# hanmekim/SceneLib2

Measured on AMD Instinct MI355X. Metric: batched MonoSLAM frames/sec (320x240, 100 feat), higher is better.
Workload: dtype f64

## Files before the change

scenelib2_amd/csrc/sl2_ekf_update.hip:

```cpp
#include "sl2_common.hpp"
#include "sl2_chol_diag.hpp"

namespace sl2 {

typedef double v4d __attribute__((ext_vector_type(4)));

__device__ __forceinline__ v4d mfma_f64(double a, double b, v4d c) {
  return __builtin_amdgcn_mfma_f64_16x16x4f64(a, b, c, 0, 0, 0);
}

#ifdef SL2_TESTING
#define SL2_EKF_TEST_SECTION 1
#include "sl2_ekf_update_testing.inc"
#undef SL2_EKF_TEST_SECTION
#endif

constexpr int kASBatch = 4;

template <int NQ, int BATCH>
__global__ void __launch_bounds__(1024) k_build_AS(const double* __restrict__ P, const double* __restrict__ f_Hx,
                                                  const double* __restrict__ f_Hy, const double* __restrict__ f_nu,
                                                  const double* __restrict__ f_R, const int* __restrict__ succ_idx,
                                                  const int* __restrict__ m_count, double* __restrict__ At,
                                                  double* __restrict__ St, const int* __restrict__ f_hcol,
                                                  const int* __restrict__ pos_err_any, int N, int ld, int mld) {
  extern __shared__ double sAt[];
  const int b = blockIdx.x;
  const int cnt = m_count[b];
  if (cnt == 0) return;
  const int m = 2 * cnt, mp = (m + 31) / 32 * 32;
  const int t = threadIdx.x;
  double* Ab = At + (size_t)b * mld * ld;
  double* Sb = St + (size_t)b * mld * mld;
  const double* Pb = P + (size_t)b * ld * ld;
// ... 101 lines not shown
  return r;
}
__device__ __forceinline__ double fast_rsqrt(double p) {
  double y = __builtin_amdgcn_rsq(p);
  y = y * __builtin_fma(-0.5 * p * y, y, 1.5);
  y = y * __builtin_fma(-0.5 * p * y, y, 1.5);
  return y;
}


#ifdef SL2_TESTING
#define SL2_EKF_TEST_SECTION 4
#include "sl2_ekf_update_testing.inc"
#undef SL2_EKF_TEST_SECTION
#endif

#ifdef SL2_TESTING
#define SL2_EKF_TEST_SECTION 5
#include "sl2_ekf_update_testing.inc"
#undef SL2_EKF_TEST_SECTION
#endif

#ifdef SL2_TESTING
#define SL2_EKF_TEST_SECTION 6
#include "sl2_ekf_update_testing.inc"
#undef SL2_EKF_TEST_SECTION
#endif


struct Tile32 {
  v4d f[2][2];
};

__device__ __forceinline__ Tile32 tile_load(const double* __restrict__ Sb, int mld, int k0, int i0, int lo, int hi) {
  Tile32 t;
#pragma unroll
  for (int kt = 0; kt < 2; ++kt)
#pragma unroll
    for (int it = 0; it < 2; ++it)
#pragma unroll
      for (int r = 0; r < 4; ++r) t.f[kt][it][r] = Sb[(size_t)(k0 + 16 * kt + hi + 4 * r) * mld + i0 + 16 * it + lo];
  return t;
}
__device__ __forceinline__ void tile_store(double* __restrict__ Sb, int mld, int k0, int i0, int lo, int hi, const Tile32& t) {
#pragma unroll
  for (int kt = 0; kt < 2; ++kt)
#pragma unroll
    for (int it = 0; it < 2; ++it)
#pragma unroll
      for (int r = 0; r < 4; ++r) Sb[(size_t)(k0 + 16 * kt + hi + 4 * r) * mld + i0 + 16 * it + lo] = t.f[kt][it][r];
}
constexpr int kTileAll = 15, kTileRowsLo = 5, kTileDiag = 11, kTileDiagLo = 1;
__device__ __forceinline__ Tile32 tile_panel(const double* sLinv, const double* __restrict__ Sb, int mld, int o, int i0, int lo,
                                             int hi, int need) {
  double b0[8], b1[8];
#pragma unroll
  for (int s8 = 0; s8 < 8; ++s8) {
    b0[s8] = Sb[(size_t)(o + 4 * s8 + hi) * mld + i0 + lo];
    b1[s8] = (need & 10) ? Sb[(size_t)(o + 4 * s8 + hi) * mld + i0 + 16 + lo] : 0.0;
  }
  Tile32 t;
#pragma unroll
  for (int kt = 0; kt < 2; ++kt)
#pragma unroll
    for (int it = 0; it < 2; ++it) t.f[kt][it] = (v4d){0, 0, 0, 0};
#pragma unroll
  for (int s8 = 0; s8 < 8; ++s8) {
    const int p = 4 * s8 + hi;
    const double a0 = sLinv[p * kLinvPitch + lo], a1 = sLinv[p * kLinvPitch + 16 + lo];
    t.f[0][0] = mfma_f64(a0, b0[s8], t.f[0][0]);
    if (need & 2) t.f[0][1] = mfma_f64(a0, b1[s8], t.f[0][1]);
    t.f[1][0] = mfma_f64(a1, b0[s8], t.f[1][0]);
    if (need & 8) t.f[1][1] = mfma_f64(a1, b1[s8], t.f[1][1]);
  }
  return t;
}
__device__ __forceinline__ Tile32 tile_panel_regs(const double* sLinv, const Tile32& in, int lo, int hi, int need) {
  Tile32 t;
#pragma unroll
  for (int kt = 0; kt < 2; ++kt)
#pragma unroll
    for (int it = 0; it < 2; ++it) t.f[kt][it] = (v4d){0, 0, 0, 0};
#pragma unroll
  for (int s8 = 0; s8 < 8; ++s8) {
    const int p = 4 * s8 + hi;
    const double a0 = sLinv[p * kLinvPitch + lo], a1 = sLinv[p * kLinvPitch + 16 + lo];
    const double b0 = in.f[s8 >> 2][0][s8 & 3], b1 = in.f[s8 >> 2][1][s8 & 3];
    t.f[0][0] = mfma_f64(a0, b0, t.f[0][0]);
    if (need & 2) t.f[0][1] = mfma_f64(a0, b1, t.f[0][1]);
    t.f[1][0] = mfma_f64(a1, b0, t.f[1][0]);
    if (need & 8) t.f[1][1] = mfma_f64(a1, b1, t.f[1][1]);
  }
  return t;
}
__device__ __forceinline__ void tile_trail(double* __restrict__ Sb, int mld, int o, int K, int I, int lo, int hi) {
  Tile32 acc = tile_load(Sb, mld, K * 32, I * 32, lo, hi);
#pragma unroll
  for (int h = 0; h < 2; ++h) {
    double a0[4], a1[4], b0[4], b1[4];
#pragma unroll
    for (int s4 = 0; s4 < 4; ++s4) {
      const size_t row = (size_t)(o + 16 * h + 4 * s4 + hi) * mld;
      a0[s4] = Sb[row + K * 32 + lo];
      a1[s4] = Sb[row + K * 32 + 16 + lo];
      b0[s4] = Sb[row + I * 32 + lo];
      b1[s4] = Sb[row + I * 32 + 16 + lo];
    }
#pragma unroll
    for (int s4 = 0; s4 < 4; ++s4) {
      acc.f[0][0] = mfma_f64(-a0[s4], b0[s4], acc.f[0][0]);
      acc.f[0][1] = mfma_f64(-a0[s4], b1[s4], acc.f[0][1]);
      acc.f[1][0] = mfma_f64(-a1[s4], b0[s4], acc.f[1][0]);
      acc.f[1][1] = mfma_f64(-a1[s4], b1[s4], acc.f[1][1]);
    }
  }
  tile_store(Sb, mld, K * 32, I * 32, lo, hi, acc);
}


#undef TR

__device__ __forceinline__ Tile32 tile_left_update(double* __restrict__ Sb, int mld, int J, int I, int kend, int lo, int hi, int need) {
  Tile32 acc = tile_load(Sb, mld, J * 32, I * 32, lo, hi);
  for (int K = 0; K < kend; ++K) {
#pragma unroll
    for (int h = 0; h < 2; ++h) {
      double a0[4], a1[4], b0[4], b1[4];
#pragma unroll
      for (int s4 = 0; s4 < 4; ++s4) {
        const size_t row = (size_t)(K * 32 + 16 * h + 4 * s4 + hi) * mld;
        a0[s4] = Sb[row + J * 32 + lo];
        a1[s4] = (need & 12) ? Sb[row + J * 32 + 16 + lo] : 0.0;
        b0[s4] = Sb[row + I * 32 + lo];
        b1[s4] = (need & 10) ? Sb[row + I * 32 + 16 + lo] : 0.0;
      }
#pragma unroll
      for (int s4 = 0; s4 < 4; ++s4) {
        acc.f[0][0] = mfma_f64(-a0[s4], b0[s4], acc.f[0][0]);
        if (need & 2) acc.f[0][1] = mfma_f64(-a0[s4], b1[s4], acc.f[0][1]);
        if (need & 4) acc.f[1][0] = mfma_f64(-a1[s4], b0[s4], acc.f[1][0]);
        if (need & 8) acc.f[1][1] = mfma_f64(-a1[s4], b1[s4], acc.f[1][1]);
      }
    }
  }
  return acc;
}
__device__ __forceinline__ void tile_diag_sub_regs(Tile32& acc, const Tile32& l, int need) {
#pragma unroll
  for (int s8 = 0; s8 < 8; ++s8) {
    const double v0 = l.f[s8 >> 2][0][s8 & 3], v1 = l.f[s8 >> 2][1][s8 & 3];
    acc.f[0][0] = mfma_f64(-v0, v0, acc.f[0][0]);
    if (need & 2) acc.f[0][1] = mfma_f64(-v0, v1, acc.f[0][1]);
    if (need & 4) acc.f[1][0] = mfma_f64(-v1, v0, acc.f[1][0]);
    if (need & 8) acc.f[1][1] = mfma_f64(-v1, v1, acc.f[1][1]);
  }
}

__global__ void __launch_bounds__(256, 4) k_chol_left(double* __restrict__ St, double* __restrict__ LinvT,
                                                      const int* __restrict__ m_count, int mld, int nblk_max, int J0, int nb_cap,
                                                      long long* trace) {
  const int b = blockIdx.x;
  const int cnt = m_count[b];
  if (cnt == 0) return;
  int nblk = (2 * cnt + 31) / 32 - J0;
  if (nblk <= 0) return;
  if (nblk > nb_cap) nblk = nb_cap;
  const int lane = threadIdx.x & 63, wave = threadIdx.x >> 6;
  const bool isD = wave == 0;
  const int mw = wave - 1;
  const bool half_last = 2 * cnt - 32 * (J0 + nblk - 1) <= 16;
  auto off_need = [&](int I) { return (half_last && I == nblk - 1) ? kTileRowsLo : kTileAll; };
  auto diag_need = [&](int I) { return (half_last && I == nblk - 1) ? kTileDiagLo : kTileDiag; };
  __shared__ double sTile[32][33];
  __shared__ double sLinv[32 * kLinvPitch];
  __shared__ double sNext[1024];
  __shared__ __attribute__((aligned(16))) double sCol[2][64];
  __shared__ double sIdent[32][33];
  double* Sb = St + (size_t)b * mld * mld + (size_t)J0 * 32 * mld + J0 * 32;
  LinvT += (size_t)J0 * 1024;
#ifdef SL2_CHOL_TRACE
#define TRL(slot) do { if (trace && lane == 0 && J < 8) trace[(((size_t)b * 4 + wave) * 8 + J) * 4 + (slot)] = (long long)__builtin_readcyclecounter(); } while (0)
#else
#define TRL(slot) do { } while (0)
#endif
#ifdef SL2_CHOL_TRACE
  if (trace && lane == 0) trace[(size_t)gridDim.x * 4 * 8 * 4 + b * 4 + wave] = __builtin_amdgcn_s_getreg(63492);
#endif
  auto diag_to_lds = [&](const Tile32& t, int lo, int hi) {
#pragma unroll
    for (int jt = 0; jt < 2; ++jt)
#pragma unroll
      for (int it = 0; it < 2; ++it)
#pragma unroll
        for (int r4 = 0; r4 < 4; ++r4) sTile[16 * it + lo][16 * jt + hi + 4 * r4] = t.f[jt][it][r4];
  };
  if (mw == 0) diag_to_lds(tile_load(Sb, mld, 0, 0, lane & 15, lane >> 4), lane & 15, lane >> 4);
  for (int i = threadIdx.x; i < 32 * 33; i += 256) (&sIdent[0][0])[i] = (i / 33 == i % 33) ? 1.0 : 0.0;
  __syncthreads();
  for (int J = 0; J < nblk; ++J) {
    const int o = J * 32;
    int lane_j = lane;
    asm volatile("" : "+v"(lane_j));
    const int lo = lane_j & 15, hi = lane_j >> 4;
    const bool more = J + 1 < nblk;
    TRL(0);
    TRL(1);
    auto solve_stored = [&](int turn) {
      for (int sidx = turn; ; sidx += 3) {
        const int t = sidx == 0 ? 3 : sidx + 4;
        if (J + t >= nblk) break;
        const Tile32 u = tile_panel(sLinv, Sb, mld, o, (J + t) * 32, lo, hi, off_need(J + t));
        tile_store(Sb, mld, o, (J + t) * 32, lo, hi, u);
      }
    };
    if (isD) {
      __builtin_amdgcn_s_setprio(3);
      const int r = lane_j & 31;
      const bool low = lane_j < 32;
      double a[32];
      const double* src = low ? &sTile[r][0] : &sIdent[r][0];
#pragma unroll
      for (int c = 0; c < 32; ++c) a[c] = src[c];
      double* rows = low ? &sTile[r][0] : &sLinv[r * kLinvPitch];
      DScal t;
      t.s = 0.0;
      d_column<0>(a, t, (unsigned)(size_t)(__attribute__((address_space(3))) double*)&sCol[0][0], &sCol[0][lane_j], rows);
      rows[31] = a[31];
      __builtin_amdgcn_s_setprio(0);
      TRL(2);
      __syncthreads();
      solve_stored(0);
    } else {
      Tile32 kept;
#pragma unroll
      for (int q = 0; q < 4; ++q) kept.f[q >> 1][q & 1] = (v4d){0, 0, 0, 0};
      int keptI = nblk;
      if (more) {
        if (mw == 1) {
          const Tile32 dn = tile_left_update(Sb, mld, J + 1, J + 1, J, lo, hi, diag_need(J + 1));
#pragma unroll
          for (int k = 0; k < 16; ++k) sNext[k * 64 + lane_j] = dn.f[k >> 3][(k >> 2) & 1][k & 3];
        }
        const int t_keep = mw == 0 ? 0 : (mw == 1 ? 4 : 2);
        for (int t = t_keep + 3; J + t < nblk; t += 3) {
          const Tile32 u = tile_left_update(Sb, mld, J, J + t, J, lo, hi, off_need(J + t));
          tile_store(Sb, mld, o, (J + t) * 32, lo, hi, u);
        }
        keptI = mw == 0 ? J + 1 : J + t_keep;
        if (keptI < nblk) kept = tile_left_update(Sb, mld, J, keptI, J, lo, hi, off_need(keptI));
      }
      TRL(2);
      __syncthreads();
      if (keptI < nblk) {
        const Tile32 l = tile_panel_regs(sLinv, kept, lo, hi, off_need(keptI));
        tile_store(Sb, mld, o, keptI * 32, lo, hi, l);
        if (mw == 0) {
          Tile32 dn;
#pragma unroll
          for (int q = 0; q < 16; ++q) dn.f[q >> 3][(q >> 2) & 1][q & 3] = sNext[q * 64 + lane_j];
          tile_diag_sub_regs(dn, l, diag_need(J + 1));
          diag_to_lds(dn, lo, hi);
        }
      }
      if (mw == 2) {
        double* Lb = LinvT + ((size_t)b * nblk_max + J) * 1024;
#pragma unroll
        for (int q = 0; q < 16; ++q) Lb[q * 64 + lane_j] = sLinv[(q * 2 + (lane_j >> 5)) * kLinvPitch + (lane_j & 31)];
      }
      if (mw >= 1) solve_stored(mw);
    }
    TRL(3);
    if (more) __syncthreads();
  }
}
#undef TRL

#ifdef SL2_TESTING
#define SL2_EKF_TEST_SECTION 8
#include "sl2_ekf_update_testing.inc"
#undef SL2_EKF_TEST_SECTION
#endif

constexpr int kFwdPitch = 48;

template <int NB>
__global__ void __launch_bounds__(256, (NB <= 8 ? 3 : 2)) k_fwdsub_lds(const double* At, double* Vt,
                                                    const double* St, const double* __restrict__ LinvT,
                                                    const int* __restrict__ m_count, int ld, int mld, int nblk_max, int B,
                                                    int J0, int col0, int ntile, int nb_cap) {
  int b, ct;
  if (!xcd_map(ntile, B, &b, &ct)) return;
  const int cnt = m_count[b];
  if (cnt == 0) return;
  int m = 2 * cnt - 32 * J0;
  if (m <= 0) return;
  if (m > 32 * nb_cap) m = 32 * nb_cap;
  const int nblk = (m + 31) / 32;
  const int tid = threadIdx.x, lane = tid & 63, wave = tid >> 6;
  const int lo = lane & 15, hi = lane >> 4;
  const int i0 = col0 + ct * 64 + wave * 16;
  const double* Ab = At + (size_t)b * mld * ld + (size_t)J0 * 32 * ld;
  double* Vb = Vt + (size_t)b * mld * ld + (size_t)J0 * 32 * ld;
  const double* Sb = St + (size_t)b * mld * mld + (size_t)J0 * 32 * mld + J0 * 32;
  const double* Lb = LinvT + ((size_t)b * nblk_max + J0) * 1024;
  __shared__ double sL[2][32 * kFwdPitch];
// ... 296 lines not shown
  const int cnt = m_count[b];
  if (cnt == 0) return;
  const int mp = (2 * cnt + 31) / 32 * 32;
  int ti = 0;
  while (t > ti) { t -= ti + 1; ++ti; }
  const int tj = t;
  const int j0 = c0 + tj * 64, i0 = c0 + ti * 64;
  if (j0 >= mp || i0 >= mp) return;
  const int tid = threadIdx.x, lane = tid & 63, wave = tid >> 6;
  const int lo = lane & 15, hi = lane >> 4;
  const int wj = (wave >> 1) * 32, wi = (wave & 1) * 32;
  double* Sb = St + (size_t)b * mld * mld;
  __shared__ double sAB[2][2][kSyrkKC * 64];
  v4d acc[2][2];
  for (int a = 0; a < 2; ++a) for (int c = 0; c < 2; ++c) acc[a][c] = (v4d){0, 0, 0, 0};
  const int kvalid = (mp - k0 < kp) ? mp - k0 : kp;
  const bool idle = (ti == tj) && (wj > wi);
  kpanel_product(Sb + (size_t)k0 * mld + j0, (size_t)mld, Sb + (size_t)k0 * mld + i0, (size_t)mld, kvalid / kSyrkKC, idle, wj, wi, sAB,
                 acc);
  if (idle) return;
#pragma unroll
  for (int a = 0; a < 2; ++a)
#pragma unroll
    for (int c = 0; c < 2; ++c)
#pragma unroll
      for (int r = 0; r < 4; ++r) {
        double* q = Sb + (size_t)(j0 + wj + 16 * a + hi + 4 * r) * mld + i0 + wi + 16 * c + lo;
        *q -= acc[a][c][r];
      }
}

constexpr int kCholPanelBlocks = 4;

static int launch_chol_panels(sl2_engine* e, int B) {
  const int pb = e->root->chol_panel == 8 ? 8 : kCholPanelBlocks;
  for (int p0 = 0; p0 < e->nblk_max; p0 += pb) {
    const int nb = e->nblk_max - p0 < pb ? e->nblk_max - p0 : pb;
    {
      LaunchScope ls(e, "k_chol_left", true);
      hipLaunchKernelGGL(k_chol_left, dim3(B), dim3(256), 0, e->stream, e->St, e->LinvT, e->m_gate, e->mld, e->nblk_max, p0, nb,
                         (long long*)nullptr);
      SL2_HIP(hipGetLastError());
    }
    const int c0 = (p0 + nb) * 32;
    if (c0 >= e->mld) break;
    const int ntile = (e->mld - c0) / 64;
    {
      LaunchScope ls(e, "k_fwdsub_lds@chol", true);
      if (pb == 8)
        hipLaunchKernelGGL((k_fwdsub_lds<8>), dim3(xcd_grid(ntile, B)), dim3(256), 0, e->stream, e->St, e->St, e->St,
                           e->LinvT, e->m_gate, e->mld, e->mld, e->nblk_max, B, p0, c0, ntile, nb);
      else
        hipLaunchKernelGGL((k_fwdsub_lds<kCholPanelBlocks>), dim3(xcd_grid(ntile, B)), dim3(256), 0, e->stream, e->St, e->St, e->St,
                           e->LinvT, e->m_gate, e->mld, e->mld, e->nblk_max, B, p0, c0, ntile, nb);
      SL2_HIP(hipGetLastError());
    }
    {
      LaunchScope ls(e, "k_chol_syrk", true);
      hipLaunchKernelGGL(k_chol_syrk, dim3(xcd_grid(ntile * (ntile + 1) / 2, B)), dim3(256), 0, e->stream, e->St, e->m_gate, e->mld,
                         B, p0 * 32, nb * 32, c0);
      SL2_HIP(hipGetLastError());
    }
  }
  return SL2_OK;
}

static int launch_fwdsub_grouped(sl2_engine* e, int B) {
  const int g = e->root->fwd_group == 4 ? 4 : 8;
  for (int J0 = 0; J0 < e->nblk_max; J0 += g) {
    if (J0 > 0) {
      LaunchScope ls(e, "k_fwd_gemm", true);
      hipLaunchKernelGGL(k_fwd_gemm, dim3(xcd_grid((g / 2) * (e->ld / 64), B)), dim3(256), 0, e->stream, e->At, e->Vt, e->St,
                         e->m_gate, e->ld, e->mld, B, J0, g / 2);
      SL2_HIP(hipGetLastError());
    }
// ... 198 lines not shown
      SL2_HIP(hipGetLastError());
    }
    {
      LaunchScope ls(e, "k_build_S");
      dim3 grid(e->mld / 32, (e->mld + 255) / 256, B);
      hipLaunchKernelGGL(k_build_S, grid, dim3(256), 0, e->stream, e->At, e->f_Hx, e->f_Hy, e->f_R, e->succ_idx, e->m_gate,
                         e->St, e->N, e->ld, e->mld);
      SL2_HIP(hipGetLastError());
    }
  } else
#endif
  {
    LaunchScope ls(e, "k_build_AS", true);
    int nsplit = B >= 1024 ? 1 : (3072 + B - 1) / B;
    if (e->root->build_split > 0) nsplit = e->root->build_split;
    if (nsplit < 1) nsplit = 1;
    const int nbatch_max = (e->N + kASBatch - 1) / kASBatch;
    if (nsplit > nbatch_max) nsplit = nbatch_max;
    if (e->ld <= 1024) {
      size_t shm = sizeof(double) * 2 * kASBatch * e->ld;
      if ((size_t)e->root->build_lds_min > shm) shm = (size_t)e->root->build_lds_min;
      hipLaunchKernelGGL((k_build_AS<1, kASBatch>), dim3(B, nsplit), dim3(e->ld), shm, e->stream, e->P, e->f_Hx, e->f_Hy, e->f_nu, e->f_R,
                         e->succ_idx, e->m_gate, e->At, e->St, e->f_hcol, e->pos_err_any, e->N, e->ld, e->mld);
    } else {
      const size_t shm = sizeof(double) * 2 * 2 * e->ld;
      hipLaunchKernelGGL((k_build_AS<2, 2>), dim3(B, nsplit), dim3(1024), shm, e->stream, e->P, e->f_Hx, e->f_Hy, e->f_nu, e->f_R,
                         e->succ_idx, e->m_gate, e->At, e->St, e->f_hcol, e->pos_err_any, e->N, e->ld, e->mld);
    }
    SL2_HIP(hipGetLastError());
  }
  if (e->nblk_max > e->root->panel_from && chol_variant >= 1 && e->mld % 64 == 0 && e->nblk_max % kCholPanelBlocks == 0) {
    int rc = launch_chol_panels(e, B);
    if (rc != SL2_OK) return rc;
  } else if (e->nblk_max <= e->root->panel_from && chol_variant == 1) {
    LaunchScope ls(e, "k_chol_left", true);
    hipLaunchKernelGGL(k_chol_left, dim3(B), dim3(256), 0, e->stream, e->St, e->LinvT, e->m_gate, e->mld, e->nblk_max, 0,
                       e->nblk_max, (long long*)e->root->chol_trace);
    SL2_HIP(hipGetLastError());
  } else {
#ifdef SL2_TESTING
    {
      for (int J = 0; J < e->nblk_max; ++J) {
        {
          LaunchScope ls(e, "k_chol_diag");
          hipLaunchKernelGGL(k_chol_diag, dim3(B), dim3(64), 0, e->stream, e->St, e->LinvT, e->m_gate, e->mld, e->nblk_max, J);
          SL2_HIP(hipGetLastError());
        }
        const int rem = e->nblk_max - 1 - J;
        if (rem > 0) {
          {
            LaunchScope ls(e, "k_chol_panel");
            hipLaunchKernelGGL(k_chol_panel, dim3(rem, B), dim3(64), 0, e->stream, e->St, e->LinvT, e->m_gate, e->mld,
                               e->nblk_max, J);
            SL2_HIP(hipGetLastError());
          }
          {
            LaunchScope ls(e, "k_chol_trail");
            hipLaunchKernelGGL(k_chol_trail, dim3(rem * (rem + 1) / 2, B), dim3(64), 0, e->stream, e->St, e->m_gate, e->mld, J);
            SL2_HIP(hipGetLastError());
          }
        }
      }
    }
#else
    set_error("launch_update: no factorisation for this system size (sl2_create should have padded it)");
    return SL2_ERR_INVALID;
#endif
  }
  {
    bool done = false;
    if (fwd_variant == 1) {
// ... 59 lines not shown
```

scenelib2_amd/csrc/sl2_ekf_update_testing.inc:

```

#if SL2_EKF_TEST_SECTION == 1
__global__ void __launch_bounds__(512) k_build_A(const double* __restrict__ P, const double* __restrict__ f_Hx,
                                                 const double* __restrict__ f_Hy, const double* __restrict__ f_nu,
                                                 const int* __restrict__ succ_idx, const int* __restrict__ m_count,
                                                 double* __restrict__ At, int N, int ld, int mld) {
  const int b = blockIdx.x;
  const int cnt = m_count[b];
  if (cnt == 0) return;
  const int cnt_pad = (cnt + 15) / 16 * 16;
  double* Ab = At + (size_t)b * mld * ld;
  const double* Pb = P + (size_t)b * ld * ld;
  for (int i = threadIdx.x; i < ld; i += blockDim.x) {
    double pc[7];
#pragma unroll
    for (int c = 0; c < 7; ++c) pc[c] = (i < 13) ? Pb[(size_t)i * ld + c] : Pb[(size_t)c * ld + i];
#pragma unroll 4
    for (int j = 0; j < cnt; ++j) {
      const int f = succ_idx[(size_t)b * N + j];
      const size_t fi = (size_t)b * N + f;
      const int pos = 13 + 3 * f;
      double py[3];
#pragma unroll
      for (int c = 0; c < 3; ++c) py[c] = Pb[(size_t)(pos + c) * ld + i];
#pragma unroll
// ... 161 lines not shown
  while (t > ri) { t -= ri + 1; ++ri; }
  const int I = J + 1 + ri, K = J + 1 + t;
  if (I >= nblk) return;
  const int lo = lane & 15, hi = lane >> 4;
  double* Sb = St + (size_t)b * mld * mld;
  v4d acc[2][2];
#pragma unroll
  for (int jt = 0; jt < 2; ++jt)
#pragma unroll
    for (int it = 0; it < 2; ++it)
#pragma unroll
      for (int r = 0; r < 4; ++r)
        acc[jt][it][r] = Sb[(size_t)(K * 32 + 16 * jt + hi + 4 * r) * mld + I * 32 + 16 * it + lo];
#pragma unroll
  for (int s = 0; s < 8; ++s) {
    const size_t row = (size_t)(J * 32 + 4 * s + hi) * mld;
    const double a0 = -Sb[row + K * 32 + lo], a1 = -Sb[row + K * 32 + 16 + lo];
    const double b0 = Sb[row + I * 32 + lo], b1 = Sb[row + I * 32 + 16 + lo];
    acc[0][0] = mfma_f64(a0, b0, acc[0][0]);
    acc[0][1] = mfma_f64(a0, b1, acc[0][1]);
    acc[1][0] = mfma_f64(a1, b0, acc[1][0]);
    acc[1][1] = mfma_f64(a1, b1, acc[1][1]);
  }
#pragma unroll
  for (int jt = 0; jt < 2; ++jt)
#pragma unroll
    for (int it = 0; it < 2; ++it)
#pragma unroll
      for (int r = 0; r < 4; ++r)
        Sb[(size_t)(K * 32 + 16 * jt + hi + 4 * r) * mld + I * 32 + 16 * it + lo] = acc[jt][it][r];
}
#endif


#if SL2_EKF_TEST_SECTION == 8
template <bool HALF>
__device__ __forceinline__ void fwd_kloop(v4d acc[2][2], const double* __restrict__ lrow, const double* vrow, int mld, int ld,
                                          int kend) {
#pragma unroll 4
  for (int kk = 0; kk < kend; kk += 4) {
    const double a0 = -lrow[(size_t)kk * mld];
    const double b0 = vrow[(size_t)kk * ld], b1 = vrow[(size_t)kk * ld + 16];
    acc[0][0] = mfma_f64(a0, b0, acc[0][0]);
    acc[0][1] = mfma_f64(a0, b1, acc[0][1]);
    if (!HALF) {
      const double a1 = -lrow[(size_t)kk * mld + 16];
      acc[1][0] = mfma_f64(a1, b0, acc[1][0]);
      acc[1][1] = mfma_f64(a1, b1, acc[1][1]);
    }
  }
}

__global__ void __launch_bounds__(128) k_fwdsub(const double* __restrict__ At, double* Vt, const double* __restrict__ St,
                                                const double* __restrict__ LinvT, const int* __restrict__ m_count, int ld,
                                                int mld, int nblk_max, int B) {
  int b, ct;
  if (!xcd_map(ld / 64, B, &b, &ct)) return;
  const int cnt = m_count[b];
  if (cnt == 0) return;
  const int m = 2 * cnt;
  const int nblk = (m + 31) / 32;
  const int lane = threadIdx.x & 63, wave = threadIdx.x >> 6;
  const int lo = lane & 15, hi = lane >> 4;
  const int i0 = ct * 64 + wave * 32;
  const double* Ab = At + (size_t)b * mld * ld;
  double* Vb = Vt + (size_t)b * mld * ld;
// ... 227 lines not shown
```

scenelib2_amd/csrc/sl2_engine.hip:

```cpp
#include "sl2_common.hpp"
#include "sl2_mapmath.hpp"

#include <mutex>

namespace sl2 {

static thread_local std::string g_err;
void set_error(const std::string& s) { g_err = s; }


__global__ void k_add_features(double* __restrict__ x, double* __restrict__ xp_org, uint8_t* __restrict__ patch,
                               int* __restrict__ patch_sums, int* __restrict__ f_flags, int* __restrict__ n_slots,
                               int* __restrict__ attempted, int* __restrict__ successful, int* __restrict__ f_label,
                               int* __restrict__ next_label, const double* __restrict__ y_in,
                               const double* __restrict__ xp_in, const uint8_t* __restrict__ patch_in, int seq0, int nfeat,
                               int N, int ld) {
  const int s = blockIdx.x, b = seq0 + s;
  const int base = n_slots[b];
  const int base_label = next_label[b];
  for (int f = threadIdx.x; f < nfeat; f += blockDim.x) {
    const int slot = base + f;
    const size_t fi = (size_t)b * N + slot;
    const size_t src = (size_t)s * nfeat + f;
    for (int k = 0; k < 3; ++k) x[(size_t)b * ld + 13 + 3 * slot + k] = y_in[src * 3 + k];
// ... 670 lines not shown
  e->search_variant = variant;
  return SL2_OK;
}

int sl2_set_search_split(sl2_engine* e, int min_bands) {
  if (!e || min_bands < 0) return SL2_ERR_INVALID;
  { int rc = drop_step_graphs(e); if (rc != SL2_OK) return rc; }
  e->search_split = min_bands;
  return SL2_OK;
}

int sl2_set_step_fusion(sl2_engine* e, int enabled) {
  if (!e) return SL2_ERR_INVALID;
  { int rc = drop_step_graphs(e); if (rc != SL2_OK) return rc; }
  e->step_fusion = enabled == 2 ? 2 : (enabled ? 1 : 0);
  return SL2_OK;
}

#ifdef SL2_CHOL_TRACE
int sl2_debug_chol_trace(sl2_engine* e, long long* out, size_t n) {
  const size_t total = (size_t)e->B * 4 * 8 * 4 + (size_t)e->B * 4;
  if (!e->chol_trace) {
    SL2_HIP(hipMalloc(&e->chol_trace, total * 8));
    SL2_HIP(hipMemset(e->chol_trace, 0, total * 8));
    return SL2_OK;
  }
  SL2_HIP(hipDeviceSynchronize());
  SL2_HIP(hipMemcpy(out, e->chol_trace, (n < total ? n : total) * 8, hipMemcpyDeviceToHost));
  return SL2_OK;
}
#endif

int sl2_set_update_variant(sl2_engine* e, int chol_variant, int fwd_variant) {
  if (!e || chol_variant < 0 || chol_variant > 1 || fwd_variant < 0 || fwd_variant > 1) return SL2_ERR_INVALID;
#ifndef SL2_TESTING
  if (chol_variant != 1 || fwd_variant != 1) {
    set_error("sl2_set_update_variant: the superseded kernel variants are compiled into the TEST build of the library only "
              "(libscenelib2_amd_test.so); this library runs chol_variant = 1, fwd_variant = 1");
    return SL2_ERR_INVALID;
  }
#endif
  { int rc = drop_step_graphs(e); if (rc != SL2_OK) return rc; }
  e->chol_variant = chol_variant;
  e->fwd_variant = fwd_variant;
  return SL2_OK;
}

int sl2_kalman_filter_predict(sl2_engine* e) {
  if (!e) return SL2_ERR_INVALID;
  SL2_HIP(hipSetDevice(e->device));
  return for_each_group(e, [](sl2_engine* g) { return launch_predict(g); });
}

int sl2_auto_select_n_features(sl2_engine* e, int n) {
  if (!e) return SL2_ERR_INVALID;
  SL2_HIP(hipSetDevice(e->device));
  return for_each_group(e, [n](sl2_engine* g) {
    int rc = launch_feature_prediction(g);
    if (rc != SL2_OK) return rc;
    return launch_select(g, n);
  });
}

int sl2_make_measurements(sl2_engine* e, const uint8_t* frames, size_t seq_stride, int frames_on_device) {
  if (!e) return SL2_ERR_INVALID;
  SL2_HIP(hipSetDevice(e->device));
  int rc = bind_frames(e, frames, seq_stride, frames_on_device);
// ... 668 lines not shown
```

Before: 1.003 million.

## Process Cholesky block columns in pairs with a role-based wave schedule

Restructures the left-looking blocked Cholesky kernel so each loop step factors two 32-wide block columns. The trailing left-update for both columns is fused (tile_left_update2 reuses each loaded B row for two accumulators), and row ownership and solver assignment now come from a new schedule header. Tile address computation is also simplified to a per-lane byte offset plus a scalar base, and the identity tile shrinks to a 64-element shifted vector. The aim is to halve the number of left-update passes over previous columns and reduce barriers and address arithmetic. The cost is more complex synchronisation, an extra LDS buffer, and higher register pressure. The old one-column kernel is kept as a test-only variant.

New measurement: 998,800. Within noise of the previous version (-0.4%).

```diff
diff --git a/scenelib2_amd/csrc/sl2_chol_schedule.hpp b/scenelib2_amd/csrc/sl2_chol_schedule.hpp
--- /dev/null
+++ b/scenelib2_amd/csrc/sl2_chol_schedule.hpp
@@ -0,0 +1,29 @@
+#pragma once
+
+#if defined(__HIPCC__) || defined(__CUDACC__)
+#define SL2_SCHED_FN __host__ __device__ inline
+#else
+#define SL2_SCHED_FN inline
+#endif
+
+namespace sl2 {
+
+constexpr int kCholRoles = 4;
+constexpr int kCholPhaseA = 0, kCholPhaseB = 1, kCholPhaseC = 2, kCholPhaseD = 3;
+
+SL2_SCHED_FN bool chol_step_is_pair(int nblk, int J) { return J + 1 < nblk; }
+SL2_SCHED_FN int chol_step_columns(int nblk, int J) { return chol_step_is_pair(nblk, J) ? 2 : 1; }
+SL2_SCHED_FN int chol_step_phases(int nblk, int J) { return chol_step_is_pair(nblk, J) ? 4 : 2; }
+SL2_SCHED_FN bool chol_barrier_after(int nblk, int J, int phase) {
+  return phase + 1 < chol_step_phases(nblk, J) || J + chol_step_columns(nblk, J) < nblk;
+}
+
+SL2_SCHED_FN int chol_row_owner(int r) { return r < 4 ? 1 + (r & 1) : (r - 4) % 3; }
+SL2_SCHED_FN bool chol_row_kept(int r) { return r < 2; }
+SL2_SCHED_FN int chol_row_solver(int phase, int r) {
+  const int s = (r - 2) % 3;
+  if (phase == kCholPhaseB) return s == 0 ? 0 : (s == 1 ? 2 : 3);
+  return s == 0 ? 0 : (s == 1 ? 3 : 1);
+}
+
+}
diff --git a/scenelib2_amd/csrc/sl2_ekf_update.hip b/scenelib2_amd/csrc/sl2_ekf_update.hip
--- a/scenelib2_amd/csrc/sl2_ekf_update.hip
+++ b/scenelib2_amd/csrc/sl2_ekf_update.hip
@@ -1,5 +1,6 @@
 #include "sl2_common.hpp"
 #include "sl2_chol_diag.hpp"
+#include "sl2_chol_schedule.hpp"
 
 namespace sl2 {
 
@@ -167,46 +168,60 @@
   v4d f[2][2];
 };
 
+__device__ __forceinline__ unsigned tile_lane_offset(int mld, int lo, int hi) {
+  unsigned v = (unsigned)(hi * mld + lo) * 8u;
+  asm volatile("" : "+v"(v));
+  return v;
+}
+__device__ __forceinline__ double& tile_at(double* base, unsigned lane_bytes) { return *(double*)((char*)base + lane_bytes); }
+__device__ __forceinline__ const double& tile_at(const double* base, unsigned lane_bytes) { return *(const double*)((const char*)base + lane_bytes); }
+
 __device__ __forceinline__ Tile32 tile_load(const double* __restrict__ Sb, int mld, int k0, int i0, int lo, int hi) {
   Tile32 t;
+  const unsigned v = tile_lane_offset(mld, lo, hi);
 #pragma unroll
   for (int kt = 0; kt < 2; ++kt)
 #pragma unroll
     for (int it = 0; it < 2; ++it)
 #pragma unroll
-      for (int r = 0; r < 4; ++r) t.f[kt][it][r] = Sb[(size_t)(k0 + 16 * kt + hi + 4 * r) * mld + i0 + 16 * it + lo];
+      for (int r = 0; r < 4; ++r) t.f[kt][it][r] = tile_at(Sb + (size_t)(k0 + 16 * kt + 4 * r) * mld + i0 + 16 * it, v);
   return t;
 }
 __device__ __forceinline__ void tile_store(double* __restrict__ Sb, int mld, int k0, int i0, int lo, int hi, const Tile32& t) {
+  const unsigned v = tile_lane_offset(mld, lo, hi);
 #pragma unroll
   for (int kt = 0; kt < 2; ++kt)
 #pragma unroll
     for (int it = 0; it < 2; ++it)
 #pragma unroll
-      for (int r = 0; r < 4; ++r) Sb[(size_t)(k0 + 16 * kt + hi + 4 * r) * mld + i0 + 16 * it + lo] = t.f[kt][it][r];
+      for (int r = 0; r < 4; ++r) tile_at(Sb + (size_t)(k0 + 16 * kt + 4 * r) * mld + i0 + 16 * it, v) = t.f[kt][it][r];
 }
 constexpr int kTileAll = 15, kTileRowsLo = 5, kTileDiag = 11, kTileDiagLo = 1;
 __device__ __forceinline__ Tile32 tile_panel(const double* sLinv, const double* __restrict__ Sb, int mld, int o, int i0, int lo,
                                              int hi, int need) {
-  double b0[8], b1[8];
-#pragma unroll
-  for (int s8 = 0; s8 < 8; ++s8) {
-    b0[s8] = Sb[(size_t)(o + 4 * s8 + hi) * mld + i0 + lo];
-    b1[s8] = (need & 10) ? Sb[(size_t)(o + 4 * s8 + hi) * mld + i0 + 16 + lo] : 0.0;
-  }
   Tile32 t;
 #pragma unroll
   for (int kt = 0; kt < 2; ++kt)
 #pragma unroll
     for (int it = 0; it < 2; ++it) t.f[kt][it] = (v4d){0, 0, 0, 0};
 #pragma unroll
-  for (int s8 = 0; s8 < 8; ++s8) {
-    const int p = 4 * s8 + hi;
-    const double a0 = sLinv[p * kLinvPitch + lo], a1 = sLinv[p * kLinvPitch + 16 + lo];
-    t.f[0][0] = mfma_f64(a0, b0[s8], t.f[0][0]);
-    if (need & 2) t.f[0][1] = mfma_f64(a0, b1[s8], t.f[0][1]);
-    t.f[1][0] = mfma_f64(a1, b0[s8], t.f[1][0]);
-    if (need & 8) t.f[1][1] = mfma_f64(a1, b1[s8], t.f[1][1]);
+  for (int h = 0; h < 2; ++h) {
+    double b0[4], b1[4];
+    const unsigned v = tile_lane_offset(mld, lo, hi);
+#pragma unroll
+    for (int s4 = 0; s4 < 4; ++s4) {
+      b0[s4] = tile_at(Sb + (size_t)(o + 16 * h + 4 * s4) * mld + i0, v);
+      b1[s4] = (need & 10) ? tile_at(Sb + (size_t)(o + 16 * h + 4 * s4) * mld + i0 + 16, v) : 0.0;
+    }
+#pragma unroll
+    for (int s4 = 0; s4 < 4; ++s4) {
+      const int p = 16 * h + 4 * s4 + hi;
+      const double a0 = sLinv[p * kLinvPitch + lo], a1 = sLinv[p * kLinvPitch + 16 + lo];
+      t.f[0][0] = mfma_f64(a0, b0[s4], t.f[0][0]);
+      if (need & 2) t.f[0][1] = mfma_f64(a0, b1[s4], t.f[0][1]);
+      t.f[1][0] = mfma_f64(a1, b0[s4], t.f[1][0]);
+      if (need & 8) t.f[1][1] = mfma_f64(a1, b1[s4], t.f[1][1]);
+    }
   }
   return t;
 }
@@ -261,13 +276,14 @@
 #pragma unroll
     for (int h = 0; h < 2; ++h) {
       double a0[4], a1[4], b0[4], b1[4];
+      const unsigned v = tile_lane_offset(mld, lo, hi);
 #pragma unroll
       for (int s4 = 0; s4 < 4; ++s4) {
-        const size_t row = (size_t)(K * 32 + 16 * h + 4 * s4 + hi) * mld;
-        a0[s4] = Sb[row + J * 32 + lo];
-        a1[s4] = (need & 12) ? Sb[row + J * 32 + 16 + lo] : 0.0;
-        b0[s4] = Sb[row + I * 32 + lo];
-        b1[s4] = (need & 10) ? Sb[row + I * 32 + 16 + lo] : 0.0;
+        const double* row = Sb + (size_t)(K * 32 + 16 * h + 4 * s4) * mld;
+        a0[s4] = tile_at(row + J * 32, v);
+        a1[s4] = (need & 12) ? tile_at(row + J * 32 + 16, v) : 0.0;
+        b0[s4] = tile_at(row + I * 32, v);
+        b1[s4] = (need & 10) ? tile_at(row + I * 32 + 16, v) : 0.0;
       }
 #pragma unroll
       for (int s4 = 0; s4 < 4; ++s4) {
@@ -289,6 +305,73 @@
     if (need & 4) acc.f[1][0] = mfma_f64(-v1, v0, acc.f[1][0]);
     if (need & 8) acc.f[1][1] = mfma_f64(-v1, v1, acc.f[1][1]);
   }
+}
+
+#ifdef SL2_TESTING
+#define SL2_EKF_TEST_SECTION 7
+#include "sl2_ekf_update_testing.inc"
+#undef SL2_EKF_TEST_SECTION
+#endif
+
+__device__ __forceinline__ void tile_left_update2(double* __restrict__ Sb, int mld, int J, int I, int lo, int hi, int need, Tile32& acc0,
+                                                  Tile32& acc1) {
+  acc0 = tile_load(Sb, mld, J * 32, I * 32, lo, hi);
+  acc1 = tile_load(Sb, mld, J * 32 + 32, I * 32, lo, hi);
+  for (int K = 0; K < J; ++K) {
+#pragma unroll
+    for (int h4 = 0; h4 < 4; ++h4) {
+      double a0[2], a1[2], c0[2], c1[2], b0[2], b1[2];
+      const unsigned voff = tile_lane_offset(mld, lo, hi);
+#pragma unroll
+      for (int s2 = 0; s2 < 2; ++s2) {
+        const double* __restrict__ rowa = Sb + (size_t)(K * 32 + 8 * h4 + 4 * s2) * mld + J * 32;
+        const double* __restrict__ rowb = Sb + (size_t)(K * 32 + 8 * h4 + 4 * s2) * mld + I * 32;
+        a0[s2] = tile_at(rowa, voff);
+        a1[s2] = tile_at(rowa + 16, voff);
+        c0[s2] = tile_at(rowa + 32, voff);
+        c1[s2] = tile_at(rowa + 48, voff);
+        b0[s2] = tile_at(rowb, voff);
+        b1[s2] = (need & 10) ? tile_at(rowb + 16, voff) : 0.0;
+      }
+#pragma unroll
+      for (int s2 = 0; s2 < 2; ++s2) {
+        acc0.f[0][0] = mfma_f64(-a0[s2], b0[s2], acc0.f[0][0]);
+        if (need & 2) acc0.f[0][1] = mfma_f64(-a0[s2], b1[s2], acc0.f[0][1]);
+        acc0.f[1][0] = mfma_f64(-a1[s2], b0[s2], acc0.f[1][0]);
+        if (need & 8) acc0.f[1][1] = mfma_f64(-a1[s2], b1[s2], acc0.f[1][1]);
+      }
+#pragma unroll
+      for (int s2 = 0; s2 < 2; ++s2) {
+        acc1.f[0][0] = mfma_f64(-c0[s2], b0[s2], acc1.f[0][0]);
+        if (need & 2) acc1.f[0][1] = mfma_f64(-c0[s2], b1[s2], acc1.f[0][1]);
+        acc1.f[1][0] = mfma_f64(-c1[s2], b0[s2], acc1.f[1][0]);
+        if (need & 8) acc1.f[1][1] = mfma_f64(-c1[s2], b1[s2], acc1.f[1][1]);
+      }
+    }
+  }
+}
+__device__ __forceinline__ void tile_pair_last(Tile32& acc, const double* sA, int lane, const Tile32& l, int need) {
+#pragma unroll
+  for (int s8 = 0; s8 < 8; ++s8) {
+    const double a0 = sA[((s8 >> 2) * 8 + (s8 & 3)) * 64 + lane], a1 = sA[((s8 >> 2) * 8 + 4 + (s8 & 3)) * 64 + lane];
+    const double b0 = l.f[s8 >> 2][0][s8 & 3], b1 = l.f[s8 >> 2][1][s8 & 3];
+    acc.f[0][0] = mfma_f64(-a0, b0, acc.f[0][0]);
+    if (need & 2) acc.f[0][1] = mfma_f64(-a0, b1, acc.f[0][1]);
+    acc.f[1][0] = mfma_f64(-a1, b0, acc.f[1][0]);
+    if (need & 8) acc.f[1][1] = mfma_f64(-a1, b1, acc.f[1][1]);
+  }
+}
+__device__ __forceinline__ Tile32 tile_load_b(const double* __restrict__ Sb, int mld, int o, int i0, int lo, int hi, int need) {
+  Tile32 t;
+  const unsigned v = tile_lane_offset(mld, lo, hi);
+#pragma unroll
+  for (int kt = 0; kt < 2; ++kt)
+#pragma unroll
+    for (int r = 0; r < 4; ++r) {
+      t.f[kt][0][r] = tile_at(Sb + (size_t)(o + 16 * kt + 4 * r) * mld + i0, v);
+      t.f[kt][1][r] = (need & 10) ? tile_at(Sb + (size_t)(o + 16 * kt + 4 * r) * mld + i0 + 16, v) : 0.0;
+    }
+  return t;
 }
 
 __global__ void __launch_bounds__(256, 4) k_chol_left(double* __restrict__ St, double* __restrict__ LinvT,
@@ -300,23 +383,22 @@
   int nblk = (2 * cnt + 31) / 32 - J0;
   if (nblk <= 0) return;
   if (nblk > nb_cap) nblk = nb_cap;
-  const int lane = threadIdx.x & 63, wave = threadIdx.x >> 6;
-  const bool isD = wave == 0;
-  const int mw = wave - 1;
+  const int lane = threadIdx.x & 63, wave0 = __builtin_amdgcn_readfirstlane(threadIdx.x >> 6);
   const bool half_last = 2 * cnt - 32 * (J0 + nblk - 1) <= 16;
   auto off_need = [&](int I) { return (half_last && I == nblk - 1) ? kTileRowsLo : kTileAll; };
   auto diag_need = [&](int I) { return (half_last && I == nblk - 1) ? kTileDiagLo : kTileDiag; };
   __shared__ double sTile[32][33];
   __shared__ double sLinv[32 * kLinvPitch];
   __shared__ double sNext[1024];
+  __shared__ double sNext2[1024];
   __shared__ __attribute__((aligned(16))) double sCol[2][64];
-  __shared__ double sIdent[32][33];
-  double* Sb = St + (size_t)b * mld * mld + (size_t)J0 * 32 * mld + J0 * 32;
+  __shared__ double sIdent[64];
+  double* Sb0 = St + (size_t)b * mld * mld + (size_t)J0 * 32 * mld + J0 * 32;
   LinvT += (size_t)J0 * 1024;
 #ifdef SL2_CHOL_TRACE
-#define TRL(slot) do { if (trace && lane == 0 && J < 8) trace[(((size_t)b * 4 + wave) * 8 + J) * 4 + (slot)] = (long long)__builtin_readcyclecounter(); } while (0)
+#define TRL(col, slot) do { if (trace && lane == 0 && (col) < 8) trace[(((size_t)b * 4 + wave) * 8 + (col)) * 4 + (slot)] = (long long)__builtin_readcyclecounter(); } while (0)
 #else
-#define TRL(slot) do { } while (0)
+#define TRL(col, slot) do { } while (0)
 #endif
 #ifdef SL2_CHOL_TRACE
   if (trace && lane == 0) trace[(size_t)gridDim.x * 4 * 8 * 4 + b * 4 + wave] = __builtin_amdgcn_s_getreg(63492);
@@ -329,31 +411,30 @@
 #pragma unroll
         for (int r4 = 0; r4 < 4; ++r4) sTile[16 * it + lo][16 * jt + hi + 4 * r4] = t.f[jt][it][r4];
   };
-  if (mw == 0) diag_to_lds(tile_load(Sb, mld, 0, 0, lane & 15, lane >> 4), lane & 15, lane >> 4);
-  for (int i = threadIdx.x; i < 32 * 33; i += 256) (&sIdent[0][0])[i] = (i / 33 == i % 33) ? 1.0 : 0.0;
+  if (wave0 == 1) diag_to_lds(tile_load(Sb0, mld, 0, 0, lane & 15, lane >> 4), lane & 15, lane >> 4);
+  if (threadIdx.x < 64) sIdent[threadIdx.x] = threadIdx.x == 31 ? 1.0 : 0.0;
   __syncthreads();
-  for (int J = 0; J < nblk; ++J) {
-    const int o = J * 32;
-    int lane_j = lane;
-    asm volatile("" : "+v"(lane_j));
-    const int lo = lane_j & 15, hi = lane_j >> 4;
-    const bool more = J + 1 < nblk;
-    TRL(0);
-    TRL(1);
-    auto solve_stored = [&](int turn) {
-      for (int sidx = turn; ; sidx += 3) {
-        const int t = sidx == 0 ? 3 : sidx + 4;
-        if (J + t >= nblk) break;
-        const Tile32 u = tile_panel(sLinv, Sb, mld, o, (J + t) * 32, lo, hi, off_need(J + t));
-        tile_store(Sb, mld, o, (J + t) * 32, lo, hi, u);
-      }
+  for (int Jstep = 0; Jstep < nblk; Jstep += 2) {
+    int J = Jstep, wave = wave0;
+    size_t step_zero = 0;
+    asm volatile("" : "+s"(J), "+s"(step_zero), "+s"(mld), "+s"(wave));
+    const bool isD = wave == 0;
+    const int mw = wave - 1;
+    double* __restrict__ Sb = Sb0 + step_zero;
+    const bool pair = chol_step_is_pair(nblk, J);
+    const int nrow = nblk - (J + 2);
+    auto fresh_lane = [&]() __attribute__((always_inline)) {
+      int l = lane;
+      asm volatile("" : "+v"(l));
+      return l;
     };
-    if (isD) {
+    auto d_factor = [&]() __attribute__((always_inline)) {
+      const int lane_j = fresh_lane();
       __builtin_amdgcn_s_setprio(3);
       const int r = lane_j & 31;
       const bool low = lane_j < 32;
       double a[32];
-      const double* src = low ? &sTile[r][0] : &sIdent[r][0];
+      const double* src = low ? &sTile[r][0] : &sIdent[31 - r];
 #pragma unroll
       for (int c = 0; c < 32; ++c) a[c] = src[c];
       double* rows = low ? &sTile[r][0] : &sLinv[r * kLinvPitch];
@@ -362,50 +443,131 @@
       d_column<0>(a, t, (unsigned)(size_t)(__attribute__((address_space(3))) double*)&sCol[0][0], &sCol[0][lane_j], rows);
       rows[31] = a[31];
       __builtin_amdgcn_s_setprio(0);
-      TRL(2);
-      __syncthreads();
-      solve_stored(0);
+    };
+    auto solve_stored = [&](int phase, int col) __attribute__((always_inline)) {
+      const int lane_j = fresh_lane(), lo = lane_j & 15, hi = lane_j >> 4;
+      for (int r = 2; r < nrow; ++r) {
+        if (chol_row_solver(phase, r) != wave) continue;
+        const int I = J + 2 + r;
+        const Tile32 u = tile_panel(sLinv, Sb, mld, col * 32, I * 32, lo, hi, off_need(I));
+        tile_store(Sb, mld, col * 32, I * 32, lo, hi, u);
+      }
+    };
+    auto linv_out = [&](int col) __attribute__((always_inline)) {
+      const int lane_j = fresh_lane();
+      double* Lb = LinvT + ((size_t)b * nblk_max + col) * 1024;
+#pragma unroll
+      for (int q = 0; q < 16; ++q) Lb[q * 64 + lane_j] = sLinv[(q * 2 + (lane_j >> 5)) * kLinvPitch + (lane_j & 31)];
+    };
+    Tile32 k0, k1;
+    auto tile_zero = [](Tile32& t) __attribute__((always_inline)) {
+#pragma unroll
+      for (int q = 0; q < 4; ++q) t.f[q >> 1][q & 1] = (v4d){0, 0, 0, 0};
+    };
+    const int keptI = J + 1 + mw;
+    const bool keeps = pair && mw >= 1 && keptI < nblk;
+
+    TRL(J, 0);
+    TRL(J, 1);
+    if (isD) {
+      d_factor();
+      tile_zero(k0);
+      tile_zero(k1);
+    } else if (pair) {
+      const int lane_j = fresh_lane(), lo = lane_j & 15, hi = lane_j >> 4;
+      for (int r = 2; r < nrow; ++r) {
+        if (chol_row_owner(r) != mw) continue;
+        Tile32 u0, u1;
+        tile_left_update2(Sb, mld, J, J + 2 + r, lo, hi, off_need(J + 2 + r), u0, u1);
+        tile_store(Sb, mld, J * 32, (J + 2 + r) * 32, lo, hi, u0);
+        tile_store(Sb, mld, J * 32 + 32, (J + 2 + r) * 32, lo, hi, u1);
+      }
+      if (mw == 0) {
+        const Tile32 dn = tile_left_update(Sb, mld, J + 1, J + 1, J, lo, hi, diag_need(J + 1));
+#pragma unroll
+        for (int q = 0; q < 16; ++q) sNext[q * 64 + lane_j] = dn.f[q >> 3][(q >> 2) & 1][q & 3];
+        k0 = tile_left_update(Sb, mld, J, J + 1, J, lo, hi, off_need(J + 1));
+        tile_zero(k1);
+      } else if (keeps) {
+        tile_left_update2(Sb, mld, J, keptI, lo, hi, off_need(keptI), k0, k1);
+      } else {
+        tile_zero(k0);
+        tile_zero(k1);
+      }
     } else {
-      Tile32 kept;
-#pragma unroll
-      for (int q = 0; q < 4; ++q) kept.f[q >> 1][q & 1] = (v4d){0, 0, 0, 0};
-      int keptI = nblk;
-      if (more) {
+      tile_zero(k0);
+      tile_zero(k1);
+    }
+    TRL(J, 2);
+    __syncthreads();
+
+    if (!isD) {
+      const int lane_j = fresh_lane(), lo = lane_j & 15, hi = lane_j >> 4;
+      if (mw == 0 && pair) {
+        k0 = tile_panel_regs(sLinv, k0, lo, hi, off_need(J + 1));
+        const Tile32& l = k0;
+        tile_store(Sb, mld, J * 32, (J + 1) * 32, lo, hi, l);
+        Tile32 dn;
+#pragma unroll
+        for (int q = 0; q < 16; ++q) dn.f[q >> 3][(q >> 2) & 1][q & 3] = sNext[q * 64 + lane_j];
+        tile_diag_sub_regs(dn, l, diag_need(J + 1));
+        diag_to_lds(dn, lo, hi);
+#pragma unroll
+        for (int q = 0; q < 16; ++q) sNext[q * 64 + lane_j] = l.f[q >> 3][(q >> 2) & 1][q & 3];
+      } else if (keeps) {
+        k0 = tile_panel_regs(sLinv, k0, lo, hi, off_need(keptI));
+        tile_store(Sb, mld, J * 32, keptI * 32, lo, hi, k0);
+      }
+      if (mw == 2) linv_out(J);
+    }
+    solve_stored(kCholPhaseB, J);
+    TRL(J, 3);
+    if (chol_barrier_after(nblk, J, kCholPhaseB)) __syncthreads();
+    if (!pair) break;
+
+    TRL(J + 1, 0);
+    TRL(J + 1, 1);
+    if (isD) {
+      d_factor();
+      tile_zero(k1);
+    } else {
+      const int lane_j = fresh_lane(), lo = lane_j & 15, hi = lane_j >> 4;
+      if (keeps) tile_pair_last(k1, sNext, lane_j, k0, off_need(keptI));
+      for (int r = 2; r < nrow; ++r) {
+        if (chol_row_owner(r) != mw) continue;
+        const int I = J + 2 + r;
+        Tile32 u = tile_load(Sb, mld, J * 32 + 32, I * 32, lo, hi);
+        tile_pair_last(u, sNext, lane_j, tile_load_b(Sb, mld, J * 32, I * 32, lo, hi, off_need(I)), off_need(I));
+        tile_store(Sb, mld, J * 32 + 32, I * 32, lo, hi, u);
+      }
+      if (mw == 0 && nrow > 0) {
+        const Tile32 dn = tile_left_update(Sb, mld, J + 2, J + 2, J + 1, lo, hi, diag_need(J + 2));
+#pragma unroll
+        for (int q = 0; q < 16; ++q) sNext2[q * 64 + lane_j] = dn.f[q >> 3][(q >> 2) & 1][q & 3];
+      }
+    }
+    TRL(J + 1, 2);
+    __syncthreads();
+
+    if (!isD) {
+      const int lane_j = fresh_lane(), lo = lane_j & 15, hi = lane_j >> 4;
+      if (keeps) {
+        k1 = tile_panel_regs(sLinv, k1, lo, hi, off_need(keptI));
+        const Tile32& l = k1;
+        tile_store(Sb, mld, J * 32 + 32, keptI * 32, lo, hi, l);
         if (mw == 1) {
-          const Tile32 dn = tile_left_update(Sb, mld, J + 1, J + 1, J, lo, hi, diag_need(J + 1));
-#pragma unroll
-          for (int k = 0; k < 16; ++k) sNext[k * 64 + lane_j] = dn.f[k >> 3][(k >> 2) & 1][k & 3];
-        }
-        const int t_keep = mw == 0 ? 0 : (mw == 1 ? 4 : 2);
-        for (int t = t_keep + 3; J + t < nblk; t += 3) {
-          const Tile32 u = tile_left_update(Sb, mld, J, J + t, J, lo, hi, off_need(J + t));
-          tile_store(Sb, mld, o, (J + t) * 32, lo, hi, u);
-        }
-        keptI = mw == 0 ? J + 1 : J + t_keep;
-        if (keptI < nblk) kept = tile_left_update(Sb, mld, J, keptI, J, lo, hi, off_need(keptI));
-      }
-      TRL(2);
-      __syncthreads();
-      if (keptI < nblk) {
-        const Tile32 l = tile_panel_regs(sLinv, kept, lo, hi, off_need(keptI));
-        tile_store(Sb, mld, o, keptI * 32, lo, hi, l);
-        if (mw == 0) {
           Tile32 dn;
 #pragma unroll
-          for (int q = 0; q < 16; ++q) dn.f[q >> 3][(q >> 2) & 1][q & 3] = sNext[q * 64 + lane_j];
-          tile_diag_sub_regs(dn, l, diag_need(J + 1));
+          for (int q = 0; q < 16; ++q) dn.f[q >> 3][(q >> 2) & 1][q & 3] = sNext2[q * 64 + lane_j];
+          tile_diag_sub_regs(dn, l, diag_need(J + 2));
           diag_to_lds(dn, lo, hi);
         }
       }
-      if (mw == 2) {
-        double* Lb = LinvT + ((size_t)b * nblk_max + J) * 1024;
-#pragma unroll
-        for (int q = 0; q < 16; ++q) Lb[q * 64 + lane_j] = sLinv[(q * 2 + (lane_j >> 5)) * kLinvPitch + (lane_j & 31)];
-      }
-      if (mw >= 1) solve_stored(mw);
-    }
-    TRL(3);
-    if (more) __syncthreads();
+      if (mw == 2) linv_out(J + 1);
+    }
+    solve_stored(kCholPhaseD, J + 1);
+    TRL(J + 1, 3);
+    if (chol_barrier_after(nblk, J, kCholPhaseD)) __syncthreads();
   }
 }
 #undef TRL
@@ -768,15 +930,28 @@
 
 constexpr int kCholPanelBlocks = 4;
 
+static int launch_chol_left(sl2_engine* e, int B, int J0, int nb, long long* trace) {
+#ifdef SL2_TESTING
+  if (e->root->chol_variant == 2) {
+    LaunchScope ls(e, "k_chol_cols1", true);
+    hipLaunchKernelGGL(k_chol_cols1, dim3(B), dim3(256), 0, e->stream, e->St, e->LinvT, e->m_gate, e->mld, e->nblk_max, J0, nb, trace);
+    SL2_HIP(hipGetLastError());
+    return SL2_OK;
+  }
+#endif
+  LaunchScope ls(e, "k_chol_left", true);
+  hipLaunchKernelGGL(k_chol_left, dim3(B), dim3(256), 0, e->stream, e->St, e->LinvT, e->m_gate, e->mld, e->nblk_max, J0, nb, trace);
+  SL2_HIP(hipGetLastError());
+  return SL2_OK;
+}
+
 static int launch_chol_panels(sl2_engine* e, int B) {
   const int pb = e->root->chol_panel == 8 ? 8 : kCholPanelBlocks;
   for (int p0 = 0; p0 < e->nblk_max; p0 += pb) {
     const int nb = e->nblk_max - p0 < pb ? e->nblk_max - p0 : pb;
     {
-      LaunchScope ls(e, "k_chol_left", true);
-      hipLaunchKernelGGL(k_chol_left, dim3(B), dim3(256), 0, e->stream, e->St, e->LinvT, e->m_gate, e->mld, e->nblk_max, p0, nb,
-                         (long long*)nullptr);
-      SL2_HIP(hipGetLastError());
+      int rc = launch_chol_left(e, B, p0, nb, nullptr);
+      if (rc != SL2_OK) return rc;
     }
     const int c0 = (p0 + nb) * 32;
     if (c0 >= e->mld) break;
@@ -1041,11 +1216,9 @@
   if (e->nblk_max > e->root->panel_from && chol_variant >= 1 && e->mld % 64 == 0 && e->nblk_max % kCholPanelBlocks == 0) {
     int rc = launch_chol_panels(e, B);
     if (rc != SL2_OK) return rc;
-  } else if (e->nblk_max <= e->root->panel_from && chol_variant == 1) {
-    LaunchScope ls(e, "k_chol_left", true);
-    hipLaunchKernelGGL(k_chol_left, dim3(B), dim3(256), 0, e->stream, e->St, e->LinvT, e->m_gate, e->mld, e->nblk_max, 0,
-                       e->nblk_max, (long long*)e->root->chol_trace);
-    SL2_HIP(hipGetLastError());
+  } else if (e->nblk_max <= e->root->panel_from && chol_variant >= 1) {
+    int rc = launch_chol_left(e, B, 0, e->nblk_max, (long long*)e->root->chol_trace);
+    if (rc != SL2_OK) return rc;
   } else {
 #ifdef SL2_TESTING
     {
diff --git a/scenelib2_amd/csrc/sl2_ekf_update_testing.inc b/scenelib2_amd/csrc/sl2_ekf_update_testing.inc
--- a/scenelib2_amd/csrc/sl2_ekf_update_testing.inc
+++ b/scenelib2_amd/csrc/sl2_ekf_update_testing.inc
@@ -217,6 +217,127 @@
 }
 #endif
 
+
+#if SL2_EKF_TEST_SECTION == 7
+__global__ void __launch_bounds__(256, 4) k_chol_cols1(double* __restrict__ St, double* __restrict__ LinvT,
+                                                       const int* __restrict__ m_count, int mld, int nblk_max, int J0, int nb_cap,
+                                                       long long* trace) {
+  const int b = blockIdx.x;
+  const int cnt = m_count[b];
+  if (cnt == 0) return;
+  int nblk = (2 * cnt + 31) / 32 - J0;
+  if (nblk <= 0) return;
+  if (nblk > nb_cap) nblk = nb_cap;
+  const int lane = threadIdx.x & 63, wave = threadIdx.x >> 6;
+  const bool isD = wave == 0;
+  const int mw = wave - 1;
+  const bool half_last = 2 * cnt - 32 * (J0 + nblk - 1) <= 16;
+  auto off_need = [&](int I) { return (half_last && I == nblk - 1) ? kTileRowsLo : kTileAll; };
+  auto diag_need = [&](int I) { return (half_last && I == nblk - 1) ? kTileDiagLo : kTileDiag; };
+  __shared__ double sTile[32][33];
+  __shared__ double sLinv[32 * kLinvPitch];
+  __shared__ double sNext[1024];
+  __shared__ __attribute__((aligned(16))) double sCol[2][64];
+  __shared__ double sIdent[32][33];
+  double* Sb = St + (size_t)b * mld * mld + (size_t)J0 * 32 * mld + J0 * 32;
+  LinvT += (size_t)J0 * 1024;
+#ifdef SL2_CHOL_TRACE
+#define TRL(slot) do { if (trace && lane == 0 && J < 8) trace[(((size_t)b * 4 + wave) * 8 + J) * 4 + (slot)] = (long long)__builtin_readcyclecounter(); } while (0)
+#else
+#define TRL(slot) do { } while (0)
+#endif
+#ifdef SL2_CHOL_TRACE
+  if (trace && lane == 0) trace[(size_t)gridDim.x * 4 * 8 * 4 + b * 4 + wave] = __builtin_amdgcn_s_getreg(63492);
+#endif
+  auto diag_to_lds = [&](const Tile32& t, int lo, int hi) {
+#pragma unroll
+    for (int jt = 0; jt < 2; ++jt)
+#pragma unroll
+      for (int it = 0; it < 2; ++it)
+#pragma unroll
+        for (int r4 = 0; r4 < 4; ++r4) sTile[16 * it + lo][16 * jt + hi + 4 * r4] = t.f[jt][it][r4];
+  };
+  if (mw == 0) diag_to_lds(tile_load(Sb, mld, 0, 0, lane & 15, lane >> 4), lane & 15, lane >> 4);
+  for (int i = threadIdx.x; i < 32 * 33; i += 256) (&sIdent[0][0])[i] = (i / 33 == i % 33) ? 1.0 : 0.0;
+  __syncthreads();
+  for (int J = 0; J < nblk; ++J) {
+    const int o = J * 32;
+    int lane_j = lane;
+    asm volatile("" : "+v"(lane_j));
+    const int lo = lane_j & 15, hi = lane_j >> 4;
+    const bool more = J + 1 < nblk;
+    TRL(0);
+    TRL(1);
+    auto solve_stored = [&](int turn) {
+      for (int sidx = turn; ; sidx += 3) {
+        const int t = sidx == 0 ? 3 : sidx + 4;
+        if (J + t >= nblk) break;
+        const Tile32 u = tile_panel(sLinv, Sb, mld, o, (J + t) * 32, lo, hi, off_need(J + t));
+        tile_store(Sb, mld, o, (J + t) * 32, lo, hi, u);
+      }
+    };
+    if (isD) {
+      __builtin_amdgcn_s_setprio(3);
+      const int r = lane_j & 31;
+      const bool low = lane_j < 32;
+      double a[32];
+      const double* src = low ? &sTile[r][0] : &sIdent[r][0];
+#pragma unroll
+      for (int c = 0; c < 32; ++c) a[c] = src[c];
+      double* rows = low ? &sTile[r][0] : &sLinv[r * kLinvPitch];
+      DScal t;
+      t.s = 0.0;
+      d_column<0>(a, t, (unsigned)(size_t)(__attribute__((address_space(3))) double*)&sCol[0][0], &sCol[0][lane_j], rows);
+      rows[31] = a[31];
+      __builtin_amdgcn_s_setprio(0);
+      TRL(2);
+      __syncthreads();
+      solve_stored(0);
+    } else {
+      Tile32 kept;
+#pragma unroll
+      for (int q = 0; q < 4; ++q) kept.f[q >> 1][q & 1] = (v4d){0, 0, 0, 0};
+      int keptI = nblk;
+      if (more) {
+        if (mw == 1) {
+          const Tile32 dn = tile_left_update(Sb, mld, J + 1, J + 1, J, lo, hi, diag_need(J + 1));
+#pragma unroll
+          for (int k = 0; k < 16; ++k) sNext[k * 64 + lane_j] = dn.f[k >> 3][(k >> 2) & 1][k & 3];
+        }
+        const int t_keep = mw == 0 ? 0 : (mw == 1 ? 4 : 2);
+        for (int t = t_keep + 3; J + t < nblk; t += 3) {
+          const Tile32 u = tile_left_update(Sb, mld, J, J + t, J, lo, hi, off_need(J + t));
+          tile_store(Sb, mld, o, (J + t) * 32, lo, hi, u);
+        }
+        keptI = mw == 0 ? J + 1 : J + t_keep;
+        if (keptI < nblk) kept = tile_left_update(Sb, mld, J, keptI, J, lo, hi, off_need(keptI));
+      }
+      TRL(2);
+      __syncthreads();
+      if (keptI < nblk) {
+        const Tile32 l = tile_panel_regs(sLinv, kept, lo, hi, off_need(keptI));
+        tile_store(Sb, mld, o, keptI * 32, lo, hi, l);
+        if (mw == 0) {
+          Tile32 dn;
+#pragma unroll
+          for (int q = 0; q < 16; ++q) dn.f[q >> 3][(q >> 2) & 1][q & 3] = sNext[q * 64 + lane_j];
+          tile_diag_sub_regs(dn, l, diag_need(J + 1));
+          diag_to_lds(dn, lo, hi);
+        }
+      }
+      if (mw == 2) {
+        double* Lb = LinvT + ((size_t)b * nblk_max + J) * 1024;
+#pragma unroll
+        for (int q = 0; q < 16; ++q) Lb[q * 64 + lane_j] = sLinv[(q * 2 + (lane_j >> 5)) * kLinvPitch + (lane_j & 31)];
+      }
+      if (mw >= 1) solve_stored(mw);
+    }
+    TRL(3);
+    if (more) __syncthreads();
+  }
+}
+#undef TRL
+#endif
 
 #if SL2_EKF_TEST_SECTION == 8
 template <bool HALF>
diff --git a/scenelib2_amd/csrc/sl2_engine.hip b/scenelib2_amd/csrc/sl2_engine.hip
--- a/scenelib2_amd/csrc/sl2_engine.hip
+++ b/scenelib2_amd/csrc/sl2_engine.hip
@@ -726,7 +726,12 @@
 #endif
 
 int sl2_set_update_variant(sl2_engine* e, int chol_variant, int fwd_variant) {
-  if (!e || chol_variant < 0 || chol_variant > 1 || fwd_variant < 0 || fwd_variant > 1) return SL2_ERR_INVALID;
+#ifdef SL2_TESTING
+  const int chol_max = 2;
+#else
+  const int chol_max = 1;
+#endif
+  if (!e || chol_variant < 0 || chol_variant > chol_max || fwd_variant < 0 || fwd_variant > 1) return SL2_ERR_INVALID;
 #ifndef SL2_TESTING
   if (chol_variant != 1 || fwd_variant != 1) {
     set_error("sl2_set_update_variant: the superseded kernel variants are compiled into the TEST build of the library only "
```
